# HueCodes/sudoku-vision

Measured on AMD Instinct MI355X. Metric: end-to-end frames/sec (1080p->81 digits), higher is better.
Workload: dtype f32

## Files before the change

include/sudoku_vision_hip.h:

```cpp
#ifndef SUDOKU_VISION_HIP_H
#define SUDOKU_VISION_HIP_H

#include <stddef.h>
#include <stdint.h>

#ifdef __cplusplus
extern "C" {
#endif

typedef struct sv_ctx sv_ctx;

typedef enum sv_status {
    SV_OK = 0,
    SV_ERR_BAD_ARG = -1,
    SV_ERR_HIP = -2,
    SV_ERR_NO_WEIGHTS = -3,
    SV_ERR_UNSUPPORTED = -4,
    SV_ERR_DEGENERATE = -5,
    SV_ERR_BUFFER = -6
} sv_status;

#define SV_CNN_PARAMS 421642
#define SV_CELLS 81
#define SV_CELL_PX 784
#define SV_CLASSES 10


int sv_version(void);
const char *sv_last_error(void);

int sv_ctx_create(int device, sv_ctx **out);
int sv_ctx_destroy(sv_ctx *ctx);

#define SV_PREC_F32 0
#define SV_PREC_BF16 1
int sv_ctx_set_precision(sv_ctx *ctx, int precision);

#define SV_CNN_AUTO 0
#define SV_CNN_F16PAIR 1
#define SV_CNN_F32MFMA 2
int sv_ctx_set_cnn_kernels(sv_ctx *ctx, int which);

int sv_ctx_reserve(sv_ctx *ctx, long max_cells);

#define SV_TIMED_KERNELS 5
int sv_timing_begin(sv_ctx *ctx);
int sv_timing_end(sv_ctx *ctx, double *ms_total , long *launches , int n_kernels);

int sv_conv_kernel_info(sv_ctx *ctx, int *algo, int *mfma_f32_conv2_per_cell, int *mfma_f32_conv1_per_cell,
                        int *mfma_f16_conv_per_cell, int *mfma_f16_fc_per_cell);

int sv_load_weights_f32(sv_ctx *ctx, const float *blob);


int sv_gray_u8(sv_ctx *ctx, const uint8_t *bgr , int n, int H, int W, ptrdiff_t pitch,
               ptrdiff_t img_stride, uint8_t *gray , void *stream);

int sv_blur_u8(sv_ctx *ctx, const uint8_t *src , int n, int H, int W, int ksize,
               uint8_t *dst , void *stream);

int sv_adaptive_threshold_u8(sv_ctx *ctx, const uint8_t *src , int n, int H, int W,
                             int block, double c, int type_inv, uint8_t *dst , void *stream);

int sv_preprocess_u8(sv_ctx *ctx, const uint8_t *bgr , int n, int H, int W, ptrdiff_t pitch,
                     ptrdiff_t img_stride, uint8_t *binary , void *stream);

int sv_preprocess_warp_cells_u8(sv_ctx *ctx, const uint8_t *bgr , int n, int H, int W, ptrdiff_t pitch, ptrdiff_t img_stride,
                                uint8_t *binary , const double *minv , uint8_t *cells , void *stream);

int sv_preprocess_bits_u8(sv_ctx *ctx, const uint8_t *bgr , int n, int H, int W, ptrdiff_t pitch,
                          ptrdiff_t img_stride, uint32_t *bits , void *stream);

int sv_despeckle_bits(sv_ctx *ctx, uint32_t *bits , int n, int H, int W, void *stream);

int sv_despeckle_u8(sv_ctx *ctx, const uint8_t *binary , int n, int H, int W,
                    uint8_t *out , uint32_t *packed , void *stream);

int sv_component_filter_bits(sv_ctx *ctx, uint32_t *bits , int n, int H, int W, double min_area_ratio, void *stream);
int sv_component_filter_u8(sv_ctx *ctx, const uint8_t *binary , int n, int H, int W, double min_area_ratio,
                           uint8_t *out , uint32_t *packed , void *stream);

long sv_sparse_bits_record_bytes(int H, int W, long cap_values);
int sv_pack_sparse_bits(sv_ctx *ctx, const uint32_t *bits , int n, int H, int W,
                        uint8_t *records , long record_stride, void *stream);

int sv_copy_to_pinned_host(sv_ctx *ctx, const void *src , void *dst_host , size_t bytes, void *stream);


int sv_find_grid_corners_u8(const uint8_t *binary , int H, int W, ptrdiff_t pitch,
                            double min_area_ratio, double epsilon_ratio, int *corners );

int sv_find_grid_corners_batch_u8(const uint8_t *binary , int n, int H, int W, ptrdiff_t pitch,
                                  ptrdiff_t img_stride, double min_area_ratio, double epsilon_ratio,
                                  int *corners , uint8_t *found , int threads);
// ... 500 lines not shown
```

sudoku-vision_amd/_native.py:

```python
import ctypes as C
import os

import numpy as np

_HERE = os.path.dirname(os.path.abspath(__file__))
LIB_PATH = os.path.join(_HERE, "csrc", "libsudokuvision_hip.so")
XCHECK_LIB_PATH = os.path.join(_HERE, "csrc", "libsudokuvision_xcheck.so")
ABI_VERSION = 2

SV_OK = 0
ERR_NAMES = {-1: "SV_ERR_BAD_ARG", -2: "SV_ERR_HIP", -3: "SV_ERR_NO_WEIGHTS", -4: "SV_ERR_UNSUPPORTED",
             -5: "SV_ERR_DEGENERATE", -6: "SV_ERR_BUFFER"}

_p, _i, _l, _d, _f, _pd = C.c_void_p, C.c_int, C.c_long, C.c_double, C.c_float, C.c_ssize_t

SIGNATURES = {
    "sv_version": [],
    "sv_last_error": [],
    "sv_ctx_create": [_i, C.POINTER(_p)],
    "sv_ctx_destroy": [_p],
    "sv_ctx_reserve": [_p, _l],
    "sv_ctx_set_precision": [_p, _i],
    "sv_load_weights_f32": [_p, _p],
    "sv_timing_begin": [_p],
    "sv_timing_end": [_p, _p, _p, _i],
    "sv_ctx_set_cnn_kernels": [_p, _i],
    "sv_conv_kernel_info": [_p, _p, _p, _p, _p, _p],
    "sv_gray_u8": [_p, _p, _i, _i, _i, _pd, _pd, _p, _p],
    "sv_blur_u8": [_p, _p, _i, _i, _i, _i, _p, _p],
    "sv_adaptive_threshold_u8": [_p, _p, _i, _i, _i, _i, _d, _i, _p, _p],
    "sv_preprocess_u8": [_p, _p, _i, _i, _i, _pd, _pd, _p, _p],
    "sv_solve_sudoku": [_p, _p, _p],
    "sv_solve_sudoku_batch": [_p, _p, _p, _i, _i, _p, _p, _p, _p],
    "sv_solve_sudoku_batch_host": [_p, _p, _i, _i, _p, _p, _p, _i],
    "sv_despeckle_u8": [_p, _p, _i, _i, _i, _p, _p, _p],
    "sv_preprocess_bits_u8": [_p, _p, _i, _i, _i, _pd, _pd, _p, _p],
    "sv_preprocess_warp_cells_u8": [_p, _p, _i, _i, _i, _pd, _pd, _p, _p, _p, _p],
    "sv_despeckle_bits": [_p, _p, _i, _i, _i, _p],
    "sv_component_filter_bits": [_p, _p, _i, _i, _i, _d, _p],
    "sv_component_filter_u8": [_p, _p, _i, _i, _i, _d, _p, _p, _p],
    "sv_copy_to_pinned_host": [_p, _p, _p, C.c_size_t, _p],
    "sv_sparse_bits_record_bytes": [_i, _i, _l],
    "sv_pack_sparse_bits": [_p, _p, _i, _i, _i, _p, _l, _p],
    "sv_find_grid_corners_sparse_batch": [_p, _l, _i, _i, _i, _d, _d, _p, _p, _i],
    "sv_sparse_bits_expand": [_p, _i, _i, _p],
    "sv_host_pool_set_affinity": [_p, _i],
    "sv_find_grid_corners_bits_batch": [_p, _i, _i, _i, _d, _d, _p, _p, _i],
    "sv_corners_to_minv": [_p, _i, _i, _f, _p],
    "sv_corners_to_minv_batch": [_p, _i, _i, _f, _p, _p],
    "sv_find_grid_corners_u8": [_p, _i, _i, _pd, _d, _d, _p],
    "sv_find_grid_corners_batch_u8": [_p, _i, _i, _i, _pd, _pd, _d, _d, _p, _p, _i],
    "sv_find_contours_u8": [_p, _i, _i, _pd, _p, _l, _p, _i, _p, _p],
    "sv_find_contours_bits": [_p, _i, _i, _p, _l, _p, _i, _p, _p],
    "sv_contour_area_i32": [_p, _i, _p],
    "sv_arc_length_i32": [_p, _i, _i, _p],
    "sv_approx_poly_dp_i32": [_p, _i, _d, _i, _p, _p],
    "sv_warp_perspective_u8": [_p, _p, _i, _i, _pd, _i, _p, _i, _p, _p],
    "sv_extract_cells_u8": [_p, _p, _i, _i, _pd, _i, _i, _i, _i, _p, _p],
    "sv_warp_cells_u8": [_p, _p, _i, _i, _i, _pd, _pd, _p, _p, _p],
    "sv_resize_linear_u8": [_p, _p, _i, _i, _pd, _p, _i, _i, _p],
    "sv_cell_ink_ratio_u8": [_p, _p, _l, _i, _p, _p, _p],
    "sv_preprocess_cells_u8": [_p, _p, _l, _p, _p],
    "sv_jpeg_parse": [_p, C.c_size_t, _p],
    "sv_jpeg_entropy_decode": [_p, C.c_size_t, _p, _p, _i],
    "sv_jpeg_entropy_decode_sparse": [_p, C.c_size_t, _p, _p, _p, _l, _p, _p, _i],
    "sv_jpeg_entropy_decode_batch": [_p, _p, _i, _p, _p, _p, _p, _p, _p, _p, _i, _p],
    "sv_jpeg_reconstruct_bgr_u8": [_p, _p, _p, _p, _p, _pd, _p],
    "sv_jpeg_reconstruct_sparse_bgr_u8": [_p, _p, _p, _p, _p, _p, _p, _pd, _p],
    "sv_jpeg_scaled_size": [_p, _i, _p, _p],
    "sv_jpeg_reconstruct_scaled_bgr_u8": [_p, _p, _p, _p, _p, _pd, _p, _i],
    "sv_jpeg_reconstruct_sparse_scaled_bgr_u8": [_p, _p, _p, _p, _p, _p, _p, _pd, _p, _i],
    "sv_jpeg_parse_luma": [_p, C.c_size_t, _p],
    "sv_jpeg_entropy_decode_luma": [_p, C.c_size_t, _p, _p, _i],
    "sv_jpeg_entropy_decode_luma_sparse": [_p, C.c_size_t, _p, _p, _p, _l, _p, _p, _i],
    "sv_jpeg_entropy_decode_luma_batch": [_p, _p, _i, _p, _p, _p, _p, _p, _p, _p, _i, _p],
    "sv_jpeg_reconstruct_gray_u8": [_p, _p, _p, _p, _p, _pd, _p, _i],
    "sv_jpeg_reconstruct_sparse_gray_u8": [_p, _p, _p, _p, _p, _p, _p, _pd, _p, _i],
    "sv_jpeg_encode_plan": [_i, _i, _i, _i, _i, _i, _p],
    "sv_jpeg_encode_bound": [_p, _l],
# ... 167 lines not shown
```

sudoku-vision_amd/csrc/k1_threshold.hip:

```cpp
#include "sv_device.h"
#include "sv_internal.h"
#include "k2_cells_body.h"

namespace {

constexpr int TW = 64, TH = 32;
constexpr int GW = TW + 14, GH = TH + 14;
constexpr int BW = TW + 10, BH = TH + 10;

struct Taps11 { float k[11]; };

__global__ __launch_bounds__(256) void k_preprocess_any(const u8 *__restrict__ bgr, int H, int W, ptrdiff_t pitch,
                                                          ptrdiff_t img_stride, u8 *__restrict__ out, Taps11 taps)
{
    __shared__ u8 g[GH][GW + 2];
    __shared__ unsigned short hb[GH][BW + 2];
    __shared__ float bl[BH][BW + 1];
    __shared__ float rw[BH][TW + 1];

    const int tid = threadIdx.x;
    const int x0 = blockIdx.x * TW, y0 = blockIdx.y * TH;
    const u8 *img = bgr + (ptrdiff_t)blockIdx.z * img_stride;
    u8 *dst = out + (ptrdiff_t)blockIdx.z * H * W;

// ... 430 lines not shown
{
    const int r = t.n / 2;
    float acc;
    if (t.n <= 5) {
        acc = __fmul_rn((float)row[x], t.k[r]);
        for (int j = 1; j <= r; j++) {
            const float pr = __fadd_rn((float)row[sv_clamp(x - j, 0, W - 1)], (float)row[sv_clamp(x + j, 0, W - 1)]);
            acc = __builtin_fmaf(pr, t.k[r + j], acc);
        }
    } else {
        acc = __fmul_rn(t.k[0], (float)row[sv_clamp(x - r, 0, W - 1)]);
        for (int j = 1; j < t.n; j++) acc = __builtin_fmaf((float)row[sv_clamp(x + j - r, 0, W - 1)], t.k[j], acc);
    }
    return acc;
}

__global__ void k_adaptive_threshold(const u8 *__restrict__ src, int H, int W, FTaps t, int idelta, int type_inv, u8 *__restrict__ dst)
{
    const int x = blockIdx.x * blockDim.x + threadIdx.x, y = blockIdx.y;
    if (x >= W) return;
    const u8 *s = src + (ptrdiff_t)blockIdx.z * H * W;
    const int r = t.n / 2;
    float acc = __fmul_rn(t.k[r], row_value(s + (ptrdiff_t)y * W, x, W, t));
    for (int j = 1; j <= r; j++) {
        const float lo = row_value(s + (ptrdiff_t)sv_clamp(y + j, 0, H - 1) * W, x, W, t);
        const float hi = row_value(s + (ptrdiff_t)sv_clamp(y - j, 0, H - 1) * W, x, W, t);
        acc = __builtin_fmaf(__fadd_rn(lo, hi), t.k[r + j], acc);
    }
    const int mean = sv_clamp(__float2int_rn(acc), 0, 255);
    const int d = (int)s[(ptrdiff_t)y * W + x] - mean;
    const bool on = type_inv ? (d <= -idelta) : (d > -idelta);
    dst[((ptrdiff_t)blockIdx.z * H + y) * W + x] = on ? 255 : 0;
}

}

static RowPairs row_pairs(const Taps11 &t)
{
    RowPairs rp;
    for (int j = 0; j < 12; j++) rp.p[j] = (f32x2_t){j < 11 ? t.k[j] : 0.f, j > 0 ? t.k[j - 1] : 0.f};
    return rp;
}

static void march_shape(int n, int H, int W, int &nstrips, int &nbands, int &TH)
{
    nstrips = (W + MARCH_STRIP - 1) / MARCH_STRIP;
    nbands = (12288 + n * nstrips - 1) / (n * nstrips);
    if (nbands > H / 32) nbands = H / 32;
    if (nbands < 1) nbands = 1;
    TH = (H + nbands - 1) / nbands;
    nbands = (H + TH - 1) / TH;
}

int svk_preprocess_bits(sv_ctx *ctx, const u8 *bgr, int n, int H, int W, ptrdiff_t pitch, ptrdiff_t img_stride, uint32_t *bits, hipStream_t s)
{
    if (H < 16 || W < 16 || (W & 31) || (pitch % 4) || (img_stride % 4) || ((uintptr_t)bgr % 4))
        return sv_fail(SV_ERR_UNSUPPORTED, "sv_preprocess_bits_u8: needs H, W >= 16, W %% 32 == 0 and a 4-byte aligned frame layout");
    Taps11 t;
    sv_gaussian_taps_f32(11, t.k);
    sv_time_scope ts(ctx, SVK_PREPROCESS, s);
    int nstrips, nbands, TH;
    march_shape(n, H, W, nstrips, nbands, TH);
    const int nitems = n * nstrips * nbands;
    hipLaunchKernelGGL(k_preprocess_march<true>, dim3((nitems + 3) / 4), dim3(256), 0, s, bgr, H, W, pitch, img_stride, (u8 *)bits, t, row_pairs(t), TH, nstrips, nbands, nitems);
    SV_LAUNCH_CHECK("k_preprocess_march<bits>");
    return SV_OK;
}

int svk_preprocess_warp_fused(sv_ctx *ctx, const u8 *bgr, int n, int H, int W, ptrdiff_t pitch, ptrdiff_t img_stride, u8 *binary, const double *minv, u8 *cells,
                              hipStream_t s)
{
    if (H < 16 || W < 16 || (W & 3) || (pitch % 4) || (img_stride % 4) || ((uintptr_t)bgr % 4) || ((uintptr_t)binary % 4))
        return sv_fail(SV_ERR_UNSUPPORTED, "sv_preprocess_warp_cells_u8: needs H, W >= 16, W %% 4 == 0 and a 4-byte aligned layout");
    Taps11 t;
    sv_gaussian_taps_f32(11, t.k);
    sv_time_scope ts(ctx, SVK_FUSED12, s);
    int nstrips, nbands, TH;
    march_shape(n, H, W, nstrips, nbands, TH);
    const long per_frame = (nstrips * nbands + 3) / 4 + 81;
    const long blocks = (long)((n + 7) / 8) * per_frame * 8;
    hipLaunchKernelGGL(k_preprocess_warp_fused, dim3((unsigned)blocks), dim3(256), 0, s, bgr, n, H, W, pitch, img_stride, binary, t, row_pairs(t), TH, nstrips, nbands, minv, cells);
    SV_LAUNCH_CHECK("k_preprocess_warp_fused");
    return SV_OK;
}

int svk_preprocess(sv_ctx *ctx, const u8 *bgr, int n, int H, int W, ptrdiff_t pitch, ptrdiff_t img_stride, u8 *binary, hipStream_t s)
{
    Taps11 t;
    sv_gaussian_taps_f32(11, t.k);
    sv_time_scope ts(ctx, SVK_PREPROCESS, s);
    if (H < 16 || W < 16) {
        dim3 grid((W + TW - 1) / TW, (H + TH - 1) / TH, n);
        hipLaunchKernelGGL(k_preprocess_any, grid, dim3(256), 0, s, bgr, H, W, pitch, img_stride, binary, t);
    } else {
        constexpr int FW = 64, FH = 64;
        const int aligned4 = (pitch % 4 == 0) && (img_stride % 4 == 0) && (W % 4 == 0) && ((uintptr_t)bgr % 4 == 0) && ((uintptr_t)binary % 4 == 0);
        dim3 grid((W + FW - 1) / FW, (H + FH - 1) / FH, n);
        if (aligned4) {
            int nstrips, nbands, TH;
            march_shape(n, H, W, nstrips, nbands, TH);
            const int nitems = n * nstrips * nbands;
            hipLaunchKernelGGL(k_preprocess_march<false>, dim3((nitems + 3) / 4), dim3(256), 0, s, bgr, H, W, pitch, img_stride, binary, t, row_pairs(t), TH, nstrips, nbands, nitems);
        } else {
            hipLaunchKernelGGL((k_preprocess_f32<64, 64, 512, 3, 2>), grid, dim3(512), 0, s, bgr, H, W, pitch, img_stride, binary, t, aligned4);
        }
    }
    SV_LAUNCH_CHECK("k_preprocess");
    return SV_OK;
}

int svk_gray(const u8 *bgr, int n, int H, int W, ptrdiff_t pitch, ptrdiff_t img_stride, u8 *gray, hipStream_t s)
{
    dim3 grid((W + 255) / 256, H, n);
    hipLaunchKernelGGL(k_gray, grid, dim3(256), 0, s, bgr, H, W, pitch, img_stride, gray);
    SV_LAUNCH_CHECK("k_gray");
    return SV_OK;
}

int svk_blur(const u8 *src, int n, int H, int W, int ksize, u8 *dst, hipStream_t s)
{
    static const int tab[4][7] = {{256, 0, 0, 0, 0, 0, 0}, {64, 128, 64, 0, 0, 0, 0}, {16, 64, 96, 64, 16, 0, 0}, {8, 28, 56, 72, 56, 28, 8}};
    FxTaps t;
    t.n = ksize;
    for (int i = 0; i < 7; i++) t.k[i] = tab[ksize / 2][i];
    dim3 grid((W + 255) / 256, H, n);
    hipLaunchKernelGGL(k_blur, grid, dim3(256), 0, s, src, H, W, t, dst);
    SV_LAUNCH_CHECK("k_blur");
    return SV_OK;
}

int svk_adaptive_threshold(const u8 *src, int n, int H, int W, int block, const float *taps, int idelta, int type_inv, u8 *dst, hipStream_t s)
{
    FTaps t;
    t.n = block;
    for (int i = 0; i < 31; i++) t.k[i] = i < block ? taps[i] : 0.f;
    dim3 grid((W + 255) / 256, H, n);
    hipLaunchKernelGGL(k_adaptive_threshold, grid, dim3(256), 0, s, src, H, W, t, idelta, type_inv, dst);
    SV_LAUNCH_CHECK("k_adaptive_threshold");
    return SV_OK;
}
```

sudoku-vision_amd/csrc/sv_api.cpp:

```cpp
#include <algorithm>
#include <cmath>
#include <cstdlib>
#include <cstring>
#include <vector>

#include "sv_augment_host.h"
#include "sv_dataset_rec.h"
#include "sv_synth_host.h"
#include "sv_internal.h"
#include "sv_philox.h"

static thread_local char g_err[512] = "";

int sv_fail(int code, const char *fmt, ...)
{
    va_list ap;
    va_start(ap, fmt);
    vsnprintf(g_err, sizeof g_err, fmt, ap);
    va_end(ap);
    return code;
}

extern "C" const char *sv_last_error(void) { return g_err; }
extern "C" int sv_version(void) { return 2; }
// ... 31 lines not shown
    free_weights(ctx->we);
    ctx->for_each_scratch([](sv_scratch &b) { b.release(); });
    for (auto &t : ctx->timeline) { (void)hipEventDestroy(t.t0); (void)hipEventDestroy(t.t1); }
    for (auto &e : ctx->event_pool) (void)hipEventDestroy(e);
    delete ctx;
    return SV_OK;
}

int sv_scratch::grow(sv_ctx *ctx, size_t bytes)
{
    if (bytes <= cap) return SV_OK;
    SV_HIP(hipSetDevice(ctx->device));
    if (p) SV_HIP(hipFree(p));
    p = nullptr;
    cap = 0;
    SV_HIP(hipMalloc(&p, bytes));
    cap = bytes;
    return SV_OK;
}

int sv_ensure_scratch(sv_ctx *ctx, long cells)
{
    if (cells <= ctx->n_cells) return SV_OK;
    ctx->n_cells = 0;
    int rc;
    if ((rc = ctx->features.grow(ctx, sizeof(float) * 3136 * (size_t)cells))) return rc;
    if ((rc = ctx->cells.grow(ctx, (size_t)SV_CELL_PX * (size_t)cells))) return rc;
    if ((rc = ctx->cells2.grow(ctx, (size_t)SV_CELL_PX * (size_t)cells))) return rc;
    ctx->n_cells = cells;
    return SV_OK;
}

static int sv_ensure_scratch_v3(sv_ctx *ctx, long cells)
{
    const long want = cells < SV_V3_SUBBATCH ? cells : SV_V3_SUBBATCH;
    if (want <= ctx->v3_cells) return SV_OK;
    ctx->v3_cells = 0;
    const int rc = ctx->v3_act.grow(ctx, svk_v3_scratch_bytes(want));
    if (rc) return rc;
    ctx->v3_cells = want;
    return SV_OK;
}

static int sv_ensure_scratch_v3_mc(sv_ctx *ctx)
{
    const int rc = sv_ensure_scratch_v3(ctx, SV_V3_SUBBATCH);
    return rc ? rc : ctx->v3_mc.grow(ctx, svk_v3_mc_scratch_bytes());
}

extern "C" int sv_ctx_set_precision(sv_ctx *ctx, int precision)
{
    if (!ctx || (precision != SV_PREC_F32 && precision != SV_PREC_BF16)) return sv_fail(SV_ERR_BAD_ARG, "sv_ctx_set_precision: bad argument");
    ctx->precision = precision;
    return SV_OK;
}

extern "C" int sv_ctx_reserve(sv_ctx *ctx, long max_cells)
{
    if (!ctx || max_cells <= 0) return sv_fail(SV_ERR_BAD_ARG, "sv_ctx_reserve: bad argument");
    SV_HIP(hipSetDevice(ctx->device));
    int rc = ctx->range_flag.grow(ctx, 2 * sizeof(int));
    if (rc || (rc = sv_ensure_scratch(ctx, max_cells))) return rc;
    return ctx->w3.loaded ? sv_ensure_scratch_v3_mc(ctx) : SV_OK;
}

sv_time_scope::sv_time_scope(sv_ctx *c, int kernel, hipStream_t st) : ctx(c), s(st)
{
    if (!ctx || !ctx->timing) return;
    hipEvent_t e[2];
    for (auto &ev : e) {
        if (!ctx->event_pool.empty()) { ev = ctx->event_pool.back(); ctx->event_pool.pop_back(); }
        else if (hipEventCreate(&ev) != hipSuccess) return;
    }
    (void)hipEventRecord(e[0], s);
    ctx->timeline.push_back({kernel, e[0], e[1]});
    idx = (int)ctx->timeline.size() - 1;
}

sv_time_scope::~sv_time_scope()
{
    if (idx >= 0) (void)hipEventRecord(ctx->timeline[idx].t1, s);
}

extern "C" int sv_timing_begin(sv_ctx *ctx)
{
    if (!ctx) return sv_fail(SV_ERR_BAD_ARG, "sv_timing_begin: NULL context");
    for (auto &t : ctx->timeline) { ctx->event_pool.push_back(t.t0); ctx->event_pool.push_back(t.t1); }
    ctx->timeline.clear();
    ctx->timing = true;
    return SV_OK;
}

extern "C" int sv_timing_end(sv_ctx *ctx, double *ms_total, long *launches, int n_kernels)
{
    if (!ctx || !ms_total || !launches || n_kernels < 0) return sv_fail(SV_ERR_BAD_ARG, "sv_timing_end: bad argument");
    ctx->timing = false;
    for (int k = 0; k < n_kernels; k++) { ms_total[k] = 0; launches[k] = 0; }
    for (auto &t : ctx->timeline) {
        SV_HIP(hipEventSynchronize(t.t1));
        float ms = 0;
        SV_HIP(hipEventElapsedTime(&ms, t.t0, t.t1));
        if (t.kernel < n_kernels) {
            ms_total[t.kernel] += ms;
            launches[t.kernel]++;
        }
        ctx->event_pool.push_back(t.t0);
// ... 1089 lines not shown
```

sudoku-vision_amd/csrc/sv_internal.h:

```cpp
#pragma once
#include <hip/hip_runtime.h>
#include <cstdarg>
#include <cstdint>
#include <cstdio>
#include <initializer_list>
#include <vector>

#include "../../include/sudoku_vision_hip.h"

typedef uint8_t u8;

struct sv_weights {
    float *conv1_w = nullptr;
    float *conv1_b = nullptr;
    float *conv2_wreg = nullptr;
    float *conv2_wino = nullptr;
    float *conv2_b = nullptr;
    float *fc1_wreg = nullptr;
    float *fc1_b = nullptr;
    unsigned short *conv2_wsplit = nullptr;
    unsigned short *conv2_bf16 = nullptr;
    unsigned short *fc1_bf16 = nullptr;
    unsigned short *conv2_h2 = nullptr;
    unsigned short *fc1_h2 = nullptr;
// ... 19 lines not shown
    std::vector<void *> allocs;
};

struct sv_weights_light {
    sv_conv3 conv[3];
    float *fc1_w = nullptr, *fc1_b = nullptr;
    float *fc2_w = nullptr, *fc2_b = nullptr;
    float temperature = 1.f;
    bool loaded = false;
    std::vector<void *> allocs;
};

struct sv_ctx;

struct sv_scratch {
    void *p = nullptr;
    size_t cap = 0;
    int grow(sv_ctx *ctx, size_t bytes);
    void release() { if (p) (void)hipFree(p); p = nullptr; cap = 0; }
    template <class T> T *as() const { return (T *)p; }
};

struct sv_ctx {
    int device = 0;
    int num_cus = 256;
    sv_weights w;
    sv_weights3 w3;
    sv_weights_light wl, we;
    sv_scratch v3_act;
    long v3_cells = 0;
    sv_scratch v3_mc;
    sv_scratch features;
    sv_scratch cells;
    sv_scratch cells2;
    long n_cells = 0;
    sv_scratch jpeg_planes;
    sv_scratch jpeg_enc;
    sv_scratch png_enc;
    sv_scratch png_dec;
    sv_scratch pp2;
    sv_scratch cc;
    sv_scratch grid2;
    sv_scratch k1_list;
    sv_scratch range_flag;
    sv_scratch overlay;
    sv_scratch eval;
    bool overlay_set = false;
    template <class F> void for_each_scratch(F f)
    {
        for (sv_scratch *b : {&v3_act, &v3_mc, &features, &cells, &cells2, &jpeg_planes, &jpeg_enc, &png_enc, &png_dec, &pp2, &cc, &grid2, &k1_list, &range_flag, &overlay, &eval}) f(*b);
    }
    int precision = 0;
    int cnn_kernels = 0;
    bool x_fc_frame = false;
    int x_motion_shape = 0;
#ifdef SV_DEV
    int dev_ablate = 0;
#endif
    bool timing = false;
    struct timed { int kernel; hipEvent_t t0, t1; };
    std::vector<timed> timeline;
    std::vector<hipEvent_t> event_pool;
};

enum sv_kernel_id { SVK_PREPROCESS = 0, SVK_WARP_CELLS = 1, SVK_CONV_FEATURES = 2, SVK_FC_HEAD = 3, SVK_FUSED12 = 4, SVK_HARRIS = 5, SVK_WARP_AFFINE = 6, SVK_COUNT = 7 };

struct sv_time_scope {
    sv_ctx *ctx; hipStream_t s; int idx = -1;
    sv_time_scope(sv_ctx *c, int kernel, hipStream_t st);
    ~sv_time_scope();
};

int sv_fail(int code, const char *fmt, ...);

#define SV_HIP(expr)                                                                         \
    do {                                                                                     \
        hipError_t e_ = (expr);                                                              \
        if (e_ != hipSuccess) return sv_fail(SV_ERR_HIP, "%s: %s", #expr, hipGetErrorString(e_)); \
    } while (0)

#define SV_LAUNCH_CHECK(name)                                                                \
    do {                                                                                     \
        hipError_t e_ = hipGetLastError();                                                   \
        if (e_ != hipSuccess) return sv_fail(SV_ERR_HIP, "launch %s: %s", name, hipGetErrorString(e_)); \
    } while (0)

#define REQUIRE_AS(fn, cond, what) \
    do { if (!(cond)) return sv_fail(SV_ERR_BAD_ARG, "%s: %s", fn, what); } while (0)
#define REQUIRE(cond, what) REQUIRE_AS(__func__, cond, what)
static inline bool frames_ok(int n, int H, int W, ptrdiff_t pitch) { return n > 0 && n < 65536 && H > 0 && W > 0 && pitch >= 3 * (ptrdiff_t)W; }
#define REQUIRE_FRAMES() REQUIRE(frames_ok(n, H, W, pitch), "bad shape")

int sv_ensure_scratch(sv_ctx *ctx, long cells);

template <class W, class T>
int sv_upload(W &w, T **dst, const T *src, size_t n)
{
    SV_HIP(hipMalloc((void **)dst, n * sizeof(T)));
    w.allocs.push_back(*dst);
    SV_HIP(hipMemcpy(*dst, src, n * sizeof(T), hipMemcpyHostToDevice));
    return SV_OK;
}

enum sv_cnn_algo { SV_ALGO_F32MFMA = 0, SV_ALGO_X_WINOGRAD = 2, SV_ALGO_X_WSPLIT = 3, SV_ALGO_F16PAIR = 4 };

struct sv_xcheck_ops {
// ... 123 lines not shown
```

sudoku-vision_amd/pipeline.py:

```python
import os
import time
from concurrent.futures import ThreadPoolExecutor
from dataclasses import dataclass, field

import numpy as np
import torch

from . import host
from .runtime import Context


def host_cpu_budget():
    n = len(os.sched_getaffinity(0)) if hasattr(os, "sched_getaffinity") else (os.cpu_count() or 1)
    for path, parse in (("/sys/fs/cgroup/cpu.max", lambda t: t.split()),
                        ("/sys/fs/cgroup/cpu/cpu.cfs_quota_us", lambda t: [t.strip(), open("/sys/fs/cgroup/cpu/cpu.cfs_period_us").read().strip()])):
        try:
            quota, period = parse(open(path).read())
            if quota not in ("max", "-1"):
                n = min(n, max(1, int(quota) // int(period)))
            break
        except (OSError, ValueError):
            continue
    return n


def _parse_cpulist(text):
    cpus = set()
    for part in text.strip().split(","):
        if part:
            lo, _, hi = part.partition("-")
            cpus.update(range(int(lo), int(hi or lo) + 1))
    return cpus


def gpu_local_cpus(device):
    try:
        p = torch.cuda.get_device_properties(device)
        path = f"/sys/bus/pci/devices/{p.pci_domain_id:04x}:{p.pci_bus_id:02x}:{p.pci_device_id:02x}.0/local_cpulist"
        cpus = _parse_cpulist(open(path).read())
    except (OSError, ValueError, AttributeError, RuntimeError):
        return None
    if hasattr(os, "sched_getaffinity"):
        cpus &= os.sched_getaffinity(0)
    return cpus or None


class FramePipeline:
    def __init__(self, ctx: Context, H: int, W: int, chunk: int = 32, host_threads=None, min_area_ratio=0.1, glue=0, despeckle=True, sparse=True, depth=5, cpu_affinity="auto", bits_direct=True,
                 quality=False, resolve=False, propagate=False, solve=False, solve_max_nodes=4096):
        self.ctx, self.H, self.W, self.chunk = ctx, H, W, chunk
        self.depth = depth = max(2, int(depth))
        self.host_threads = host_threads or max(1, host_cpu_budget() - 2)
        self.min_area_ratio = min_area_ratio
        self.despeckle = bool(despeckle) and min_area_ratio * H * W > 61 * 61
        self.glue = glue
        dev = ctx.device
        self.s_pre = torch.cuda.Stream(dev)
        self.s_d2h = torch.cuda.Stream(dev)
        self.s_cls = torch.cuda.Stream(dev)
        self.packed = self.despeckle and W % 32 == 0
        self.bits_direct = bool(bits_direct)
        self.sparse = self.packed and bool(sparse) and H * ((W // 32 + 63) // 64) <= 16000
        if self.packed:
            self.dev_bits = [torch.empty((chunk, H, W // 32), dtype=torch.int32, device=dev) for _ in range(depth)]
        if self.sparse:
            cap = H * (W // 32) // 3 if sparse is True else int(sparse)
            self.rec_bytes = host.sparse_bits_record_bytes(H, W, cap)
            self.pinned = [torch.empty((chunk, self.rec_bytes), dtype=torch.uint8).pin_memory() for _ in range(depth)]
            self.dev_rec = [torch.empty((chunk, self.rec_bytes), dtype=torch.uint8, device=dev) for _ in range(depth)]
            self.s_side = torch.cuda.Stream(dev)
        elif self.packed:
            self.pinned = [torch.empty((chunk, H, W // 32), dtype=torch.int32).pin_memory() for _ in range(depth)]
        else:
            self.pinned = [torch.empty((chunk, H, W), dtype=torch.uint8).pin_memory() for _ in range(depth)]
        self.dev_bin = None
        self.minv_pin = [torch.empty((chunk, 9), dtype=torch.float64).pin_memory() for _ in range(depth)]
        self.minv_dev = [torch.empty((chunk, 9), dtype=torch.float64, device=dev) for _ in range(depth)]
        self.cpus = gpu_local_cpus(dev) if cpu_affinity == "auto" else (set(cpu_affinity) if cpu_affinity else None)
        if self.cpus:
            host.set_pool_affinity(self.cpus)
        self.pool = ThreadPoolExecutor(1, initializer=(lambda: os.sched_setaffinity(0, self.cpus)) if self.cpus and hasattr(os, "sched_setaffinity") else None)
        self.dense_fallbacks = 0
        self.quality = bool(quality)
        if self.quality:
            self.q_bin = [None] * depth
        self.resolve = bool(resolve)
        self.propagate = bool(propagate)
        self.solve, self.solve_max_nodes = bool(solve), int(solve_max_nodes)
        ctx.reserve(chunk * 81)

    def _search(self, slot, m, ev):
        ev.synchronize()
        if self.sparse:
            corners, found = host.find_grid_corners_sparse_batch(self.pinned[slot][:m].numpy(), self.H, self.W, self.min_area_ratio, 0.02, self.host_threads)
            over = np.nonzero(found == 2)[0]
            if over.size:
                with torch.cuda.stream(self.s_side):
                    dense = self.dev_bits[slot][torch.from_numpy(over).to(self.ctx.device)].cpu().numpy()
                c2, f2 = host.find_grid_corners_bits_batch(dense, self.H, self.W, self.min_area_ratio, 0.02, self.host_threads)
                corners[over], found[over] = c2, f2
                self.dense_fallbacks += int(over.size)
            found = found.astype(bool)
        elif self.packed:
            corners, found = host.find_grid_corners_bits_batch(self.pinned[slot][:m].numpy(), self.H, self.W, self.min_area_ratio, 0.02, self.host_threads)
        else:
            corners, found = host.find_grid_corners_batch(self.pinned[slot][:m].numpy(), self.min_area_ratio, 0.02, self.host_threads)
        minv, ok = Context.corners_to_minv_batch(corners.astype(np.float32))
        self.minv_pin[slot][:m] = torch.from_numpy(minv.reshape(m, 9))
        return corners, found & ok

    def describe(self):
        d2h = (f"pinned D2H of sparse records of the bit-packed binary (row masks + non-zero words, {self.rec_bytes // 1000} KB/frame over PCIe, "
               f"dense fallback {self.H * self.W // 8 // 1000} KB)" if self.sparse
               else f"pinned D2H of the bit-packed binary ({self.H * self.W // 8 // 1000} KB/frame over PCIe)" if self.packed
               else f"pinned D2H of the binary ({self.H * self.W // 1000} KB/frame over PCIe)")
        k1 = ("K1 (bit image) -> despeckle in place (exact speck filter) -> " if self.packed and self.bits_direct
              else f"K1 -> {'despeckle (exact speck filter) -> ' if self.despeckle else ''}")
        return (f"{k1}{d2h} -> C++ contour corner search on "
                f"{self.host_threads} host threads -> K2 -> K3, {self.chunk}-frame chunks, {self.depth} in flight"
                + (f", host threads on the GPU's NUMA node ({len(self.cpus)} CPUs)" if self.cpus else "")
                + (", then top-3 -> K9 (validation + beam-search conflict repair) per chunk" if self.resolve else "")
                + (", then K10 (constraint propagation) per chunk" if self.propagate else "")
                + (f", then K14 (solver, {self.solve_max_nodes} search nodes per frame at most) per chunk" if self.solve else ""))

    def run(self, frames, out=None, repeat=1, total=None):
        n = frames.shape[0]
        if (repeat > 1 or total is not None) and n % self.chunk:
            raise ValueError("repeat / total need the chunk size to divide the number of frames")
        dev = self.ctx.device
        if out is None:
            out = {"logits": torch.empty((n, 81, 10), dtype=torch.float32, device=dev),
                   "digits": torch.empty((n, 81), dtype=torch.uint8, device=dev),
                   "conf": torch.empty((n, 81), dtype=torch.float32, device=dev)}
        corners_all = np.zeros((n, 4, 2), np.int32)
        found_all = np.zeros(n, bool)
        cur = torch.cuda.current_stream(dev)
        self.s_pre.wait_stream(cur)
        self.s_d2h.wait_stream(cur)
        self.s_cls.wait_stream(cur)
        bits_direct = (self.packed and self.bits_direct and frames.is_contiguous() and frames.data_ptr() % 4 == 0 and (3 * self.W) % 4 == 0
                       and self.H >= 16 and self.W >= 16)
        if not bits_direct and self.dev_bin is None:
            self.dev_bin = [torch.empty((self.chunk, self.H, self.W), dtype=torch.uint8, device=dev) for _ in range(self.depth)]
        if self.quality:
            qshape, qtype = ((self.chunk, self.H, self.W // 32), torch.int32) if bits_direct else ((self.chunk, self.H, self.W), torch.uint8)
            if self.q_bin[0] is None or tuple(self.q_bin[0].shape) != qshape or self.q_bin[0].dtype != qtype:
                self.q_bin = [torch.empty(qshape, dtype=qtype, device=dev) for _ in range(self.depth)]
            q_s1 = torch.empty((n,), dtype=torch.int64, device=dev)
            q_s2 = torch.empty((n,), dtype=torch.int64, device=dev)
            q_hist = torch.empty((n, 256), dtype=torch.int32, device=dev)
            q_cnt = torch.zeros((n, 20), dtype=torch.int32, device=dev)
        if self.resolve:
            resolve_ok = torch.empty((n,), dtype=torch.uint8, device=dev)
            out.update(resolved_digits=torch.empty((n, 81), dtype=torch.uint8, device=dev), resolve_success=resolve_ok.view(torch.bool),
                       num_conflicts=torch.empty((n,), dtype=torch.int32, device=dev), n_corrections=torch.empty((n,), dtype=torch.uint8, device=dev))
        if self.propagate:
            propagate_ok = torch.empty((n,), dtype=torch.uint8, device=dev)
            out.update(propagated_digits=torch.empty((n, 81), dtype=torch.uint8, device=dev), propagate_valid=propagate_ok.view(torch.bool),
                       contradiction_cell=torch.empty((n,), dtype=torch.uint8, device=dev), n_propagated=torch.empty((n,), dtype=torch.uint8, device=dev))
        if self.solve:
            solve_in = out["propagated_digits" if self.propagate else "resolved_digits" if self.resolve else "digits"]
            out.update(solution=torch.empty((n, 81), dtype=torch.uint8, device=dev), solve_result=torch.empty((n,), dtype=torch.int8, device=dev),
                       solve_nodes=torch.empty((n,), dtype=torch.int32, device=dev))
        if total is None:
            starts = [(s0, min(self.chunk, n - s0)) for _ in range(repeat) for s0 in range(0, n, self.chunk)]
        else:
            starts = [((k * self.chunk) % n, min(self.chunk, total - k * self.chunk)) for k in range((total + self.chunk - 1) // self.chunk)]
        pending = []
        free_ev = [None] * self.depth

        def classify(item):
            fut, slot, s, m = item
            corners, found = fut.result()
            corners_all[s:s + m], found_all[s:s + m] = corners, found
            with torch.cuda.stream(self.s_cls):
                self.minv_dev[slot][:m].copy_(self.minv_pin[slot][:m], non_blocking=True)
                sub = {k: out[k][s:s + m] for k in ("logits", "digits", "conf")}
                self.ctx.frames_to_digits(frames[s:s + m], self.minv_dev[slot][:m], out=sub, glue=self.glue)
                if self.quality:
                    self.ctx.grid_line_coverage(self.q_bin[slot][:m], self.minv_dev[slot][:m], out=q_cnt[s:s + m])
                if self.resolve:
                    idx, prob = self.ctx.softmax_topk(sub["logits"], 3)
                    self.ctx.resolve_conflicts(idx.view(m, 81, 3), prob.view(m, 81, 3), acceptance_rule=True,
                                               out={"digits": out["resolved_digits"][s:s + m], "success": resolve_ok[s:s + m],
                                                    "num_conflicts_after": out["num_conflicts"][s:s + m], "n_corrections": out["n_corrections"][s:s + m]})
                if self.propagate:
                    self.ctx.propagate_constraints(out["resolved_digits" if self.resolve else "digits"][s:s + m],
                                                   out={"grid": out["propagated_digits"][s:s + m], "is_valid": propagate_ok[s:s + m],
                                                        "contradiction_cell": out["contradiction_cell"][s:s + m], "n_resolved": out["n_propagated"][s:s + m]})
                lost = None
                if not found.all():
                    lost = torch.from_numpy(~found).to(dev)
                    out["digits"][s:s + m][lost] = 0
                    if self.propagate:
                        out["propagated_digits"][s:s + m][lost] = 0
                        out["n_propagated"][s:s + m][lost] = 0
                        out["contradiction_cell"][s:s + m][lost] = 255
                        propagate_ok[s:s + m][lost] = 0
                    if self.resolve:
                        for key in ("resolved_digits", "num_conflicts", "n_corrections"):
                            out[key][s:s + m][lost] = 0
                        resolve_ok[s:s + m][lost] = 0
                if self.solve:
                    self.ctx.solve_sudoku(solve_in[s:s + m], propagate_ok[s:s + m] if self.propagate else None if lost is None else ~lost,
                                          max_nodes=self.solve_max_nodes,
                                          out={"solution": out["solution"][s:s + m], "result": out["solve_result"][s:s + m], "nodes": out["solve_nodes"][s:s + m]})
                ev = torch.cuda.Event(blocking=True)
                ev.record(self.s_cls)
                free_ev[slot] = ev

        for i, (s, m) in enumerate(starts):
            slot = i % self.depth
            if free_ev[slot] is not None:
                free_ev[slot].synchronize()
            with torch.cuda.stream(self.s_pre):
                if bits_direct:
                    b = self.ctx.preprocess_bits(frames[s:s + m], out=self.dev_bits[slot][:m])
                    if self.quality:
                        self.q_bin[slot][:m].copy_(b)
                    b = self.ctx.despeckle_bits(b)
                else:
                    b = self.ctx.preprocess(frames[s:s + m], out=self.dev_bin[slot][:m])
                    if self.quality:
                        self.q_bin[slot][:m].copy_(b)
                if self.packed:
                    if not bits_direct:
                        b = self.ctx.despeckle(b, out=b, packed=self.dev_bits[slot][:m])
                    if self.sparse:
                        b = self.ctx.pack_sparse_bits(b, self.dev_rec[slot])
                elif self.despeckle:
                    b = self.ctx.despeckle(b, out=b)
                ready = torch.cuda.Event()
                ready.record(self.s_pre)
                if self.quality:
                    self.ctx.frame_quality_stats(frames[s:s + m], out=(q_s1[s:s + m], q_s2[s:s + m], q_hist[s:s + m]))
            with torch.cuda.stream(self.s_d2h):
                self.s_d2h.wait_event(ready)
                self.pinned[slot][:m].copy_(b, non_blocking=True)
                ev = torch.cuda.Event(blocking=True)
                ev.record(self.s_d2h)
            pending.append((self.pool.submit(self._search, slot, m, ev), slot, s, m))
            if len(pending) > self.depth - 2:
                classify(pending.pop(0))
        while pending:
            classify(pending.pop(0))
        cur.wait_stream(self.s_cls)
        out["corners"], out["found"] = corners_all, found_all
        if self.quality:
            from .cv.grid_quality import scores_from_stats
            cur.wait_stream(self.s_pre)
            s1, s2, hist, cnt = (t.cpu().numpy() for t in (q_s1, q_s2, q_hist, q_cnt))
            out["quality"] = scores_from_stats(s1, s2, hist, cnt, corners_all, found_all, self.H * self.W).astype(np.float32)
        return out


def _corners_behind_filters(ctx, frames, binary_dev=None, min_area_ratio=0.1):
    H, W = frames.shape[1], frames.shape[2]
    k4 = min_area_ratio * H * W > 61 * 61
    if W % 32 == 0 and H >= 16:
        if binary_dev is None:
            bits = ctx.preprocess_bits(frames)
            if k4:
                ctx.despeckle_bits(bits)
        else:
            bits = torch.empty((1, H, W // 32), dtype=torch.int32, device=ctx.device)
            if k4:
                ctx.despeckle(binary_dev[None], packed=bits)
            else:
                ctx.component_filter(binary_dev[None], 0.0, packed=bits)
        ctx.component_filter_bits(bits, min_area_ratio)
        corners, found = host.find_grid_corners_bits_batch(bits.cpu().numpy(), H, W, min_area_ratio, threads=1)
        return corners[0] if found[0] else None
    b = (ctx.preprocess(frames) if binary_dev is None else binary_dev[None].contiguous())
    if k4:
        b = ctx.despeckle(b)
    b = ctx.component_filter(b, min_area_ratio, out=b if k4 or binary_dev is None else None)
    return host.find_grid_corners(b[0].cpu().numpy(), min_area_ratio)


def recognize_image(image, model_state_dict=None, ctx=None, glue=Context.GLUE_RUNPY, top_k=0, quality=False, preprocess="v1", model="v1", resolve=False, propagate=False, component_filter=False, grid="v1", solve=False, overlay=False):
    from .runtime import default_context
    if overlay and not solve:
        raise ValueError("overlay=True needs solve=True: there is nothing to draw without a solution")
    if grid not in ("v1", "v2"):
        raise ValueError(f"grid must be 'v1' or 'v2', got {grid!r}")
    if preprocess not in ("v1", "v2"):
        raise ValueError(f"preprocess must be 'v1' or 'v2', got {preprocess!r}")
# ... 330 lines not shown
```

sudoku-vision_amd/runtime.py:

```python
import ctypes as C
import threading

import numpy as np
import torch

from . import _native

_V1_LAYOUT = (("conv1.weight", (32, 1, 3, 3)), ("conv1.bias", (32,)), ("conv2.weight", (64, 32, 3, 3)), ("conv2.bias", (64,)),
              ("fc1.weight", (128, 3136)), ("fc1.bias", (128,)), ("fc2.weight", (10, 128)), ("fc2.bias", (10,)))


_V3_BLOCKS = ((32, 32, 1), (32, 64, 2), (64, 64, 1), (64, 128, 2), (128, 128, 1))


def v3_layout(use_se=True):
    def bn(prefix, c):
        return [(f"{prefix}.{n}", (c,)) for n in ("weight", "bias", "running_mean", "running_var")]
    out = [("temperature", (1,)), ("stem.0.weight", (32, 1, 3, 3))] + bn("stem.1", 32)
    for i, (cin, c, stride) in enumerate(_V3_BLOCKS, 1):
        L = f"layer{i}"
        out += [(f"{L}.conv1.weight", (c, cin, 3, 3))] + bn(f"{L}.bn1", c) + [(f"{L}.conv2.weight", (c, c, 3, 3))] + bn(f"{L}.bn2", c)
        if use_se:
            out += [(f"{L}.se.excite.0.weight", (c // 4, c)), (f"{L}.se.excite.2.weight", (c, c // 4))]
        if stride != 1 or cin != c:
# ... 76 lines not shown
    return img, st[0]


def _batch_layout(x, device, name, ch):
    _dev_tensor(x, name, torch.uint8, device, shape=(None, None, None, ch) if ch > 1 else (None, None, None))
    n, H, row = x.shape[0], x.shape[1], x.shape[2] * ch
    st = x.stride()
    if not (st[-1] == 1 and st[2] == ch and st[1] >= row and (n == 1 or st[0] >= st[1] * (H - 1) + row)):
        x = x.contiguous()
        st = x.stride()
    return x, st[1], (st[0] if n > 1 else st[1] * H)


def _frame_layout(frames, device):
    return _batch_layout(frames, device, "frames", 3)


def _plane_layout(x, device, name="gray"):
    return _batch_layout(x, device, name, 1)


def _to_dev(a, ctx):
    if isinstance(a, torch.Tensor):
        if a.dtype != torch.uint8 or not a.is_cuda:
            raise TypeError("expected a uint8 CUDA tensor or a numpy uint8 array")
        return a, True
    a = np.asarray(a)
    if a.dtype != np.uint8:
        raise TypeError(f"expected uint8 image, got {a.dtype}")
    return torch.from_numpy(np.ascontiguousarray(a)).to(ctx.device), False


def _back(t, was_tensor):
    return t if was_tensor else t.cpu().numpy()


def _model_context(x, training, name, eval_note):
    if training:
        raise NotImplementedError(f"{name} (MI355X): inference only -- call .eval() ({eval_note} in eval mode)")
    if not x.is_cuda:
        raise RuntimeError(f"{name} (MI355X): input must be a CUDA tensor; there is no CPU fallback")
    if x.dim() != 4 or tuple(x.shape[1:]) != (1, 28, 28):
        raise ValueError(f"expected input of shape (batch, 1, 28, 28), got {tuple(x.shape)}")
    return default_context(x.device)


class Context:
    def __init__(self, device=None, library=None):
        _require_gpu()
        self.device = torch.device("cuda", torch.cuda.current_device() if device is None else torch.device(device).index or 0)
        self._lib = library or _native.lib()
        self._h = C.c_void_p()
        self._check(self._lib.sv_ctx_create(self.device.index, C.byref(self._h)), "sv_ctx_create")
        self._weights_key = None
        self._weights_v3_key = None
        self._weights_light_key = None
        self._weights_empty_key = None

    def _check(self, rc, what):
        _native.check(rc, what, self._lib)

    def _out(self, t, shape, dtype, name):
        if t is None:
            return torch.empty(tuple(shape), dtype=dtype, device=self.device)
        if not isinstance(t, torch.Tensor) or tuple(t.shape) != tuple(shape) or t.dtype != dtype or not t.is_contiguous() or t.device != self.device:
            raise TypeError(f"{name} must be a contiguous {dtype} tensor of shape {list(shape)} on {self.device}")
        return t

    def _minv(self, minv_dev, n):
        _dev_tensor(minv_dev, "minv_dev", torch.float64, self.device)
        if minv_dev.numel() != 9 * n:
            raise ValueError(f"minv_dev must hold {n} 3x3 matrices, got shape {list(minv_dev.shape)}")
        return minv_dev.contiguous()

    def close(self):
        if self._h:
            self._lib.sv_ctx_destroy(self._h)
            self._h = C.c_void_p()

    def __del__(self):
        try:
            self.close()
        except Exception:
            pass

    def load_state_dict(self, sd, key=None):
        blob = _state_blob(sd, _V1_LAYOUT, "DigitCNN")
        self._check(self._lib.sv_load_weights_f32(self._h, blob.ctypes.data_as(C.c_void_p)), "sv_load_weights_f32")
        self._weights_key = key

    def load_state_dict_v3(self, sd, use_se=None, key=None):
        has_se = any(".se.excite." in k for k in sd)
        if use_se is None:
            use_se = has_se
        elif bool(use_se) != has_se:
            raise ValueError(f"use_se={use_se} but the state_dict {'has' if has_se else 'has no'} se.excite weights")
        blob = _state_blob(sd, v3_layout(bool(use_se)), "DigitCNNv3", strict=True)
        self._check(self._lib.sv_load_weights_v3_f32(self._h, blob.ctypes.data_as(C.c_void_p), blob.size, int(bool(use_se))), "sv_load_weights_v3_f32")
        self._weights_v3_key = key

    def load_state_dict_v3_light(self, sd, key=None):
        blob = _state_blob(sd, light_layout(), "DigitCNNv3Light", strict=True)
        self._check(self._lib.sv_load_weights_v3_light_f32(self._h, blob.ctypes.data_as(C.c_void_p), blob.size), "sv_load_weights_v3_light_f32")
        self._weights_light_key = key

    def load_state_dict_empty(self, sd, key=None):
        blob = _state_blob(sd, empty_layout(), "EmptyClassifier", strict=True)
        self._check(self._lib.sv_load_weights_empty_f32(self._h, blob.ctypes.data_as(C.c_void_p), blob.size), "sv_load_weights_empty_f32")
        self._weights_empty_key = key

    PREC_F32, PREC_BF16 = 0, 1

    def set_precision(self, precision):
        self._check(self._lib.sv_ctx_set_precision(self._h, int(precision)), "sv_ctx_set_precision")

    CNN_AUTO, CNN_F16PAIR, CNN_F32MFMA = 0, 1, 2
    CNN_X_WINOGRAD, CNN_X_WSPLIT = 102, 103

    def set_cnn_kernels(self, which):
        self._check(self._lib.sv_ctx_set_cnn_kernels(self._h, int(which)), "sv_ctx_set_cnn_kernels")

    def reserve(self, max_cells):
        self._check(self._lib.sv_ctx_reserve(self._h, int(max_cells)), "sv_ctx_reserve")

    KERNELS = ("k_preprocess", "k_warp_cells", "k_conv_features", "k_fc_head", "k_preprocess_warp_fused", "k_harris", "k_warp_affine")

    def timing_begin(self):
        self._check(self._lib.sv_timing_begin(self._h), "sv_timing_begin")

    def timing_end(self):
        ms = (C.c_double * len(self.KERNELS))()
        cnt = (C.c_long * len(self.KERNELS))()
        self._check(self._lib.sv_timing_end(self._h, ms, cnt, len(self.KERNELS)), "sv_timing_end")
        return {k: (ms[i], cnt[i]) for i, k in enumerate(self.KERNELS)}

    CONV_ALGO_NAMES = {0: "k_conv_features_pc + k_fc_head (direct implicit GEMM, f32 MFMA)",
                       2: "k_conv_features_wstream (Winograd F(2x2,3x3), f32 MFMA; cross-check build)",
                       3: "k_conv_features_wsplit (Winograd, bf16 MFMA with 3-way operand split; cross-check build)",
                       4: "k_conv_features_h2 + k_fc_head_h2p (f16 hi/lo operand pairs, f16 MFMA, f32 accumulation)"}

    def conv_kernel_info(self):
        v = [C.c_int() for _ in range(5)]
        self._check(self._lib.sv_conv_kernel_info(self._h, *[C.byref(x) for x in v]), "sv_conv_kernel_info")
        a = v[0].value
        return {"algo": a, "name": self.CONV_ALGO_NAMES.get(a, str(a)), "mfma_conv2": v[1].value, "mfma_conv1": v[2].value,
                "mfma_f16_conv": v[3].value, "mfma_f16_fc": v[4].value}

    def gray(self, bgr):
        bgr, pitch, fstride = _frame_layout(bgr, self.device)
        n, H, W = bgr.shape[0], bgr.shape[1], bgr.shape[2]
        out = torch.empty((n, H, W), dtype=torch.uint8, device=self.device)
        self._check(self._lib.sv_gray_u8(self._h, _ptr(bgr), n, H, W, pitch, fstride, _ptr(out), _stream_ptr()), "sv_gray_u8")
        return out

    def blur(self, gray, ksize):
        gray = _dev_tensor(gray, "gray", torch.uint8, self.device, ndim=3).contiguous()
        n, H, W = gray.shape
        out = torch.empty_like(gray)
        self._check(self._lib.sv_blur_u8(self._h, _ptr(gray), n, H, W, int(ksize), _ptr(out), _stream_ptr()), "sv_blur_u8")
        return out

    def adaptive_threshold(self, gray, block_size, c, inv=True):
        gray = _dev_tensor(gray, "gray", torch.uint8, self.device, ndim=3).contiguous()
        n, H, W = gray.shape
        out = torch.empty_like(gray)
        self._check(self._lib.sv_adaptive_threshold_u8(self._h, _ptr(gray), n, H, W, int(block_size), float(c), int(bool(inv)),
                                                             _ptr(out), _stream_ptr()), "sv_adaptive_threshold_u8")
        return out

    def preprocess(self, frames, out=None):
        frames, pitch, fstride = _frame_layout(frames, self.device)
        n, H, W = frames.shape[0], frames.shape[1], frames.shape[2]
        out = self._out(out, (n, H, W), torch.uint8, "out")
# ... 1141 lines not shown
```

Baseline: 202,900.

## Run despeckle on a high-priority stream and cap K1 occupancy via LDS padding

Moves despeckle and bit-packing off the K1 preprocess stream onto a separate high-priority stream, so one chunk's filtering can overlap the next chunk's K1. The classifier stream is also made high priority. To leave compute units free for those overlapping kernels, K1 gets 9 KB of extra dynamic LDS when set to 3 waves per SIMD, which limits its occupancy. Shadow mode is on by default, which adds a cross-stream event per chunk. The lower K1 occupancy could slow K1 itself if the overlap does not make up for it.

```diff
diff --git a/include/sudoku_vision_hip.h b/include/sudoku_vision_hip.h
--- a/include/sudoku_vision_hip.h
+++ b/include/sudoku_vision_hip.h
@@ -40,6 +40,8 @@
 #define SV_CNN_F16PAIR 1
 #define SV_CNN_F32MFMA 2
 int sv_ctx_set_cnn_kernels(sv_ctx *ctx, int which);
+
+int sv_ctx_set_k1_occupancy(sv_ctx *ctx, int waves_per_simd);
 
 int sv_ctx_reserve(sv_ctx *ctx, long max_cells);
 
diff --git a/sudoku-vision_amd/_native.py b/sudoku-vision_amd/_native.py
--- a/sudoku-vision_amd/_native.py
+++ b/sudoku-vision_amd/_native.py
@@ -25,6 +25,7 @@
     "sv_timing_begin": [_p],
     "sv_timing_end": [_p, _p, _p, _i],
     "sv_ctx_set_cnn_kernels": [_p, _i],
+    "sv_ctx_set_k1_occupancy": [_p, _i],
     "sv_conv_kernel_info": [_p, _p, _p, _p, _p, _p],
     "sv_gray_u8": [_p, _p, _i, _i, _i, _pd, _pd, _p, _p],
     "sv_blur_u8": [_p, _p, _i, _i, _i, _i, _p, _p],
diff --git a/sudoku-vision_amd/csrc/k1_threshold.hip b/sudoku-vision_amd/csrc/k1_threshold.hip
--- a/sudoku-vision_amd/csrc/k1_threshold.hip
+++ b/sudoku-vision_amd/csrc/k1_threshold.hip
@@ -506,6 +506,8 @@
     nbands = (H + TH - 1) / TH;
 }
 
+static unsigned march_lds_pad(const sv_ctx *ctx) { return ctx && ctx->k1_waves == 3 ? 9u * 1024u : 0u; }
+
 int svk_preprocess_bits(sv_ctx *ctx, const u8 *bgr, int n, int H, int W, ptrdiff_t pitch, ptrdiff_t img_stride, uint32_t *bits, hipStream_t s)
 {
     if (H < 16 || W < 16 || (W & 31) || (pitch % 4) || (img_stride % 4) || ((uintptr_t)bgr % 4))
@@ -516,7 +518,7 @@
     int nstrips, nbands, TH;
     march_shape(n, H, W, nstrips, nbands, TH);
     const int nitems = n * nstrips * nbands;
-    hipLaunchKernelGGL(k_preprocess_march<true>, dim3((nitems + 3) / 4), dim3(256), 0, s, bgr, H, W, pitch, img_stride, (u8 *)bits, t, row_pairs(t), TH, nstrips, nbands, nitems);
+    hipLaunchKernelGGL(k_preprocess_march<true>, dim3((nitems + 3) / 4), dim3(256), march_lds_pad(ctx), s, bgr, H, W, pitch, img_stride, (u8 *)bits, t, row_pairs(t), TH, nstrips, nbands, nitems);
     SV_LAUNCH_CHECK("k_preprocess_march<bits>");
     return SV_OK;
 }
@@ -554,7 +556,7 @@
             int nstrips, nbands, TH;
             march_shape(n, H, W, nstrips, nbands, TH);
             const int nitems = n * nstrips * nbands;
-            hipLaunchKernelGGL(k_preprocess_march<false>, dim3((nitems + 3) / 4), dim3(256), 0, s, bgr, H, W, pitch, img_stride, binary, t, row_pairs(t), TH, nstrips, nbands, nitems);
+            hipLaunchKernelGGL(k_preprocess_march<false>, dim3((nitems + 3) / 4), dim3(256), march_lds_pad(ctx), s, bgr, H, W, pitch, img_stride, binary, t, row_pairs(t), TH, nstrips, nbands, nitems);
         } else {
             hipLaunchKernelGGL((k_preprocess_f32<64, 64, 512, 3, 2>), grid, dim3(512), 0, s, bgr, H, W, pitch, img_stride, binary, t, aligned4);
         }
diff --git a/sudoku-vision_amd/csrc/sv_api.cpp b/sudoku-vision_amd/csrc/sv_api.cpp
--- a/sudoku-vision_amd/csrc/sv_api.cpp
+++ b/sudoku-vision_amd/csrc/sv_api.cpp
@@ -107,6 +107,14 @@
 {
     if (!ctx || (precision != SV_PREC_F32 && precision != SV_PREC_BF16)) return sv_fail(SV_ERR_BAD_ARG, "sv_ctx_set_precision: bad argument");
     ctx->precision = precision;
+    return SV_OK;
+}
+
+extern "C" int sv_ctx_set_k1_occupancy(sv_ctx *ctx, int waves_per_simd)
+{
+    if (!ctx) return sv_fail(SV_ERR_BAD_ARG, "sv_ctx_set_k1_occupancy: NULL context");
+    if (waves_per_simd != 3 && waves_per_simd != 4) return sv_fail(SV_ERR_BAD_ARG, "sv_ctx_set_k1_occupancy: %d waves per SIMD (3 or 4)", waves_per_simd);
+    ctx->k1_waves = waves_per_simd;
     return SV_OK;
 }
 
diff --git a/sudoku-vision_amd/csrc/sv_internal.h b/sudoku-vision_amd/csrc/sv_internal.h
--- a/sudoku-vision_amd/csrc/sv_internal.h
+++ b/sudoku-vision_amd/csrc/sv_internal.h
@@ -95,6 +95,7 @@
     }
     int precision = 0;
     int cnn_kernels = 0;
+    int k1_waves = 4;
     bool x_fc_frame = false;
     int x_motion_shape = 0;
 #ifdef SV_DEV
diff --git a/sudoku-vision_amd/pipeline.py b/sudoku-vision_amd/pipeline.py
--- a/sudoku-vision_amd/pipeline.py
+++ b/sudoku-vision_amd/pipeline.py
@@ -47,7 +47,7 @@
 
 class FramePipeline:
     def __init__(self, ctx: Context, H: int, W: int, chunk: int = 32, host_threads=None, min_area_ratio=0.1, glue=0, despeckle=True, sparse=True, depth=5, cpu_affinity="auto", bits_direct=True,
-                 quality=False, resolve=False, propagate=False, solve=False, solve_max_nodes=4096):
+                 quality=False, resolve=False, propagate=False, solve=False, solve_max_nodes=4096, shadow=True, k1_occupancy=None):
         self.ctx, self.H, self.W, self.chunk = ctx, H, W, chunk
         self.depth = depth = max(2, int(depth))
         self.host_threads = host_threads or max(1, host_cpu_budget() - 2)
@@ -55,9 +55,13 @@
         self.despeckle = bool(despeckle) and min_area_ratio * H * W > 61 * 61
         self.glue = glue
         dev = ctx.device
+        self.shadow = bool(shadow)
+        self.k1_occupancy = int(k1_occupancy) if k1_occupancy else (3 if self.shadow else 4)
+        hi = {"priority": -1} if self.shadow else {}
         self.s_pre = torch.cuda.Stream(dev)
+        self.s_flt = torch.cuda.Stream(dev, **hi) if self.shadow else self.s_pre
         self.s_d2h = torch.cuda.Stream(dev)
-        self.s_cls = torch.cuda.Stream(dev)
+        self.s_cls = torch.cuda.Stream(dev, **hi)
         self.packed = self.despeckle and W % 32 == 0
         self.bits_direct = bool(bits_direct)
         self.sparse = self.packed and bool(sparse) and H * ((W // 32 + 63) // 64) <= 16000
@@ -116,14 +120,25 @@
                else f"pinned D2H of the binary ({self.H * self.W // 1000} KB/frame over PCIe)")
         k1 = ("K1 (bit image) -> despeckle in place (exact speck filter) -> " if self.packed and self.bits_direct
               else f"K1 -> {'despeckle (exact speck filter) -> ' if self.despeckle else ''}")
+        streams = (f"K1 at {self.k1_occupancy} waves per SIMD on its own stream, despeckle + pack on a high-priority stream beside the next chunk's K1, "
+                   "D2H on a third, K2 -> K3 on a high-priority fourth" if self.shadow
+                   else f"K1 at {self.k1_occupancy} waves per SIMD -> despeckle -> pack on one stream, D2H on a second, K2 -> K3 on a third")
         return (f"{k1}{d2h} -> C++ contour corner search on "
-                f"{self.host_threads} host threads -> K2 -> K3, {self.chunk}-frame chunks, {self.depth} in flight"
+                f"{self.host_threads} host threads -> K2 -> K3, {self.chunk}-frame chunks, {self.depth} in flight; streams: {streams}"
                 + (f", host threads on the GPU's NUMA node ({len(self.cpus)} CPUs)" if self.cpus else "")
                 + (", then top-3 -> K9 (validation + beam-search conflict repair) per chunk" if self.resolve else "")
                 + (", then K10 (constraint propagation) per chunk" if self.propagate else "")
                 + (f", then K14 (solver, {self.solve_max_nodes} search nodes per frame at most) per chunk" if self.solve else ""))
 
     def run(self, frames, out=None, repeat=1, total=None):
+        before = self.ctx.k1_occupancy
+        self.ctx.set_k1_occupancy(self.k1_occupancy)
+        try:
+            return self._run(frames, out, repeat, total)
+        finally:
+            self.ctx.set_k1_occupancy(before)
+
+    def _run(self, frames, out, repeat, total):
         n = frames.shape[0]
         if (repeat > 1 or total is not None) and n % self.chunk:
             raise ValueError("repeat / total need the chunk size to divide the number of frames")
@@ -136,6 +151,7 @@
         found_all = np.zeros(n, bool)
         cur = torch.cuda.current_stream(dev)
         self.s_pre.wait_stream(cur)
+        self.s_flt.wait_stream(cur)
         self.s_d2h.wait_stream(cur)
         self.s_cls.wait_stream(cur)
         bits_direct = (self.packed and self.bits_direct and frames.is_contiguous() and frames.data_ptr() % 4 == 0 and (3 * self.W) % 4 == 0
@@ -218,11 +234,18 @@
                     b = self.ctx.preprocess_bits(frames[s:s + m], out=self.dev_bits[slot][:m])
                     if self.quality:
                         self.q_bin[slot][:m].copy_(b)
-                    b = self.ctx.despeckle_bits(b)
                 else:
                     b = self.ctx.preprocess(frames[s:s + m], out=self.dev_bin[slot][:m])
                     if self.quality:
                         self.q_bin[slot][:m].copy_(b)
+                if self.s_flt is not self.s_pre:
+                    k1_done = torch.cuda.Event()
+                    k1_done.record(self.s_pre)
+            with torch.cuda.stream(self.s_flt):
+                if self.s_flt is not self.s_pre:
+                    self.s_flt.wait_event(k1_done)
+                if bits_direct:
+                    b = self.ctx.despeckle_bits(b)
                 if self.packed:
                     if not bits_direct:
                         b = self.ctx.despeckle(b, out=b, packed=self.dev_bits[slot][:m])
@@ -231,8 +254,9 @@
                 elif self.despeckle:
                     b = self.ctx.despeckle(b, out=b)
                 ready = torch.cuda.Event()
-                ready.record(self.s_pre)
-                if self.quality:
+                ready.record(self.s_flt)
+            if self.quality:
+                with torch.cuda.stream(self.s_pre):
                     self.ctx.frame_quality_stats(frames[s:s + m], out=(q_s1[s:s + m], q_s2[s:s + m], q_hist[s:s + m]))
             with torch.cuda.stream(self.s_d2h):
                 self.s_d2h.wait_event(ready)
diff --git a/sudoku-vision_amd/runtime.py b/sudoku-vision_amd/runtime.py
--- a/sudoku-vision_amd/runtime.py
+++ b/sudoku-vision_amd/runtime.py
@@ -152,6 +152,7 @@
         self._lib = library or _native.lib()
         self._h = C.c_void_p()
         self._check(self._lib.sv_ctx_create(self.device.index, C.byref(self._h)), "sv_ctx_create")
+        self.k1_occupancy = 4
         self._weights_key = None
         self._weights_v3_key = None
         self._weights_light_key = None
@@ -219,6 +220,10 @@
 
     def set_cnn_kernels(self, which):
         self._check(self._lib.sv_ctx_set_cnn_kernels(self._h, int(which)), "sv_ctx_set_cnn_kernels")
+
+    def set_k1_occupancy(self, waves_per_simd):
+        self._check(self._lib.sv_ctx_set_k1_occupancy(self._h, int(waves_per_simd)), "sv_ctx_set_k1_occupancy")
+        self.k1_occupancy = int(waves_per_simd)
 
     def reserve(self, max_cells):
         self._check(self._lib.sv_ctx_reserve(self._h, int(max_cells)), "sv_ctx_reserve")
```

Result: slower. 194,100 (-4.3%).
